# FlinkML/flink-parameter-server

Hardware: NVIDIA H100
Metric: matrix-factorization updates/sec (whole box, max over ranks) (higher is better)
Workload: dtype fp32

## Files before the change

### flink-parameter-server_b200/models/mf/device.py

```python
from __future__ import annotations

import math
import os
from typing import Iterable, Optional, Sequence, Tuple

import torch
import torch.distributed as dist

from ...errors import FactorIsNotANumberException
from ...ops import native
from ...utils.metrics import GLOBAL as METRICS
from ...runtime.device_stream import DevicePrefetcher
from ...store.replica_cache import ReplicaCache
from ...store.sharded_table import ShardedTable

ERR_SIGMOID = 0
ERR_PLAIN = 1

DEFAULT_DEVICE_PULL_LIMIT = 0

L2_TABLE_BYTES = 48 << 20
WINDOW_BUDGET = 256 << 20
WINDOW_BYTES_PER_ROW = 8 + 12
WINDOW_MAX_STRIDE = 128
# ... 89 lines not shown
                 output_ring=None, loss: str = "pointwise", regularization: float = 0.0,
                 step_window: Optional[int] = None, optimizer: str = "sgd",
                 negative_sampling: str = "uniform", margin: Optional[float] = None):
        self._pending = []
        self.step_window = 0
        check_negative_sampling(negative_sampling, negative_sample_rate)
        self.negative_sampling = negative_sampling
        if loss not in ("pointwise", "bpr", "warp"):
            raise ValueError(f"loss must be 'pointwise', 'bpr' or 'warp', got {loss!r}")
        self.loss, self.reg = loss, float(regularization)
        if loss == "pointwise" and self.reg != 0.0:
            raise ValueError("regularization is only supported with loss='bpr' or loss='warp'")
        self.margin = check_warp(loss, margin, optimizer=optimizer, negative_sampling=negative_sampling)
        if loss != "pointwise":
            if output_ring is not None:
                raise ValueError(f"the per-update output ring is not supported with loss={loss!r}")
            if kernel == "tma":
                raise ValueError(f"kernel='tma' is not supported with loss={loss!r}")
            if item_blocking:
                raise ValueError(f"item_blocking is not supported with loss={loss!r}")
            item_blocking = False
        self.device = torch.cuda.current_device() if device is None else int(device)
        self.cuda_device = torch.device("cuda", self.device)
        self.group = group
        ready = dist.is_available() and dist.is_initialized()
        self.world = dist.get_world_size(group) if ready else 1
        self.rank = dist.get_rank(group) if ready else 0
        if item_cache is None:
            item_cache = self.world > 1 and os.environ.get("FPS_ITEM_CACHE", "1") != "0"
        check_optimizer(optimizer, item_cache=bool(item_cache), output_ring=output_ring, kernel=kernel)
        self.optimizer = optimizer
        self.num_users, self.num_items, self.k = int(num_users), int(num_items), int(num_factors)
        self.lr = float(learning_rate)
        self.neg = int(negative_sample_rate)
        self.pull_limit = int(pull_limit)
        self.err_mode = int(err_mode)
        self.seed = int(seed)
        self.step_no = 0
        self.kernel = kernel
        self.credits = (torch.tensor([self.pull_limit, 0], dtype=torch.int32, device=self.cuda_device)
                        if self.pull_limit >= 32 and os.environ.get("FPS_STATIC_LIMITER", "0") != "1"
                        and loss == "pointwise" and optimizer == "sgd" else None)
        self.output_ring = output_ring
        with torch.cuda.device(self.device):
            self._items = ShardedTable(num_items, num_factors, partition="hash", group=group,
                                      device=self.device, init="uniform",
                                      init_range=(range_min, range_max), seed=seed * 2 + 1,
                                      track_touched=track_touched)
            n_local = -(-self.num_users // self.world)
            self._users = torch.empty((n_local, self._items.stride), dtype=torch.float32,
                                     device=self.cuda_device)
            native.init_rows(self._users, self.k, self.rank, self.world, native.PART_HASH, n_local,
                             seed * 2 + 2, range_min, range_max)
            self._stats = torch.zeros(STATS_SIZE[loss], dtype=torch.float32, device=self.cuda_device)
            self._user_acc = self._item_acc = None
            if optimizer == "adagrad":
                self._user_acc = torch.zeros(n_local, dtype=torch.float32, device=self.cuda_device)
                self._item_acc = self._items.row_accumulators()
            self._nan_flag = torch.zeros(1, dtype=torch.int32, device=self.cuda_device)
            self.user_memory = int(user_memory) if self.neg > 0 else 0
            if self.user_memory > 0:
                self.seen = torch.full((n_local, self.user_memory), -1, dtype=torch.int32,
                                       device=self.cuda_device)
                self.seen_pos = torch.zeros(n_local, dtype=torch.int32, device=self.cuda_device)
            self._registry = (native.seen_registry(self.num_items, self.cuda_device)
                              if negative_sampling == "seen" else None)
        self.item_cache = bool(item_cache)
        self.sync_every = max(1, int(sync_every))
        self.sync_interval_ms = sync_interval_ms
        self.flush_count, self.flush_require = flush_count, flush_require
        self._own_inplace = replica_own_inplace
        self.replica = (ReplicaCache(self._items, self.sync_every, sync_interval_ms,
                                     require=flush_require, flush_count=flush_count,
                                     own_inplace=replica_own_inplace)
                        if self.item_cache else None)
        row_bytes = self._items.stride * 4
        if item_blocking is None:
            item_blocking = ((self.world == 1 or self.item_cache) and self.num_items * row_bytes > (48 << 20)
                             and (self.neg == 0 or self.user_memory > 0 or negative_sampling == "seen")
                             and os.environ.get("FPS_ITEM_BLOCKING", "1") != "0")
        self.item_blocking = bool(item_blocking)
        block_bytes = int(os.environ.get("FPS_BLOCK_BYTES", block_bytes))
        self.l2_hints = self.item_blocking and os.environ.get("FPS_L2_HINTS", "0") == "1"
        per_bucket = max(1, int(block_bytes) // row_bytes)
        self.block_shift = max(0, per_bucket.bit_length() - 1)
        table_rows = self._items.rows_per_shard * self.world if self.item_cache else self.num_items
        self._table_rows = table_rows
        while -(-table_rows >> self.block_shift) > native.BUCKET_MAX:
            self.block_shift += 1
        self.block_buckets = max(1, -(-table_rows >> self.block_shift))
        if self.item_blocking:
            with torch.cuda.device(self.device):
                self._bucket_scratch = torch.zeros(2 * native.BUCKET_MAX, dtype=torch.int32,
                                                   device=self.cuda_device)
        self.step_window = step_window_size(step_window, world=self.world, item_cache=self.item_cache,
                                            loss=self.loss, table_rows=self.num_items, stride=self._items.stride,
                                            env=os.environ.get("FPS_STEP_WINDOW"), optimizer=optimizer)
        self._win = None
        self._win_phase_ns = None
        self._graph_capture = False
        self._per_launch = False
        self._items.barrier()

    @property
    def stats(self) -> torch.Tensor:
        self._drain()
        return self._stats

    @property
    def users(self) -> torch.Tensor:
        self._drain()
        return self._users

    @property
    def items(self) -> ShardedTable:
        self._drain()
        return self._items

    @property
    def nan_flag(self) -> torch.Tensor:
        self._drain()
        return self._nan_flag

    @property
    def accumulators(self) -> Optional[Tuple[torch.Tensor, torch.Tensor]]:
        self._drain()
        if self._item_acc is None:
            return None
        return self._user_acc, self._item_acc.local

    def _windowable(self, users, items, ratings) -> bool:
        if self.step_window < 2 or self._graph_capture or self._per_launch:
            return False
        packed = items is None
        return step_windowable(
            neg=self.neg, output_ring=self.output_ring, pull_limit=self.pull_limit, credits=self.credits,
            kernel=self.kernel, kernel_env=os.environ.get("FPS_MF_KERNEL", "reg"),
            reg_variant_env=os.environ.get("FPS_MF_REG_VARIANT"), l2_hints=self.l2_hints, packed=packed,
            dtypes=(users.dtype,) if packed else (users.dtype, items.dtype, ratings.dtype),
            n_records=users.numel(), table_rows=self.num_items, on_gpu=users.is_cuda,
            capturing=torch.cuda.is_current_stream_capturing())

    def _stage(self, users, items, ratings) -> None:
        if self._win is None:
            rows, w = self.num_items, self.step_window
            slot_bytes = -(-rows * 12 // 256) * 256
            with torch.cuda.device(self.device):
                dev = self.cuda_device
                self._win = {
                    "slot_bytes": slot_bytes,
                    "stage": torch.empty(w * slot_bytes, dtype=torch.uint8, device=dev),
                    "slots": torch.full((w, rows), -1, dtype=torch.int64, device=dev),
                    "user_bits": torch.zeros(-(-self._users.shape[0] // 32), dtype=torch.int32, device=dev),
                    "ctl": torch.zeros(2 * native.WINDOW_MAX, dtype=torch.int32, device=dev),
                    "slot_stats": torch.zeros((w, 2), dtype=torch.float32, device=dev),
                }
        j = len(self._pending)
        n = users.numel()
        sb = self._win["slot_bytes"]
        slot = self._win["stage"][j * sb:(j + 1) * sb]
        if items is None:
            slot[:8 * n].view(torch.int64).copy_(users.reshape(-1), non_blocking=True)
        else:
            ids = slot[:12 * n].view(torch.int32)
            ids[:n].copy_(users.reshape(-1), non_blocking=True)
            ids[n:2 * n].copy_(items.reshape(-1), non_blocking=True)
            ids[2 * n:].view(torch.float32).copy_(ratings.reshape(-1), non_blocking=True)
        self._pending.append((n, 1 if items is None else 0))
        self.step_no += 1
        METRICS.inc("mf_ratings", n)

    def _drain(self) -> int:
        n = len(self._pending)
        if n == 0:
            return 0
        counts, fmts = zip(*self._pending)
        self._pending = []
        w = self._win
        native.mf_window_drain(w["stage"], w["slot_bytes"], counts, fmts, self._users, self._items.local, self.lr,
                               self.err_mode, w["slots"], w["user_bits"], w["ctl"], self._stats, w["slot_stats"],
                               self._nan_flag, phase_ns=self._win_phase_ns)
        return n

    def flush(self) -> None:
        self._drain()
        if self.replica is not None:
            self.replica.flush()

    def step(self, users: torch.Tensor, items: Optional[torch.Tensor] = None,
             ratings: Optional[torch.Tensor] = None, negatives: Optional[torch.Tensor] = None) -> None:
        if self.loss == "pointwise" and negatives is None and self._windowable(users, items, ratings):
            self._stage(users, items, ratings)
            if len(self._pending) >= self.step_window:
                self._drain()
            return
        self._drain()
        check_negative_sampling(self.negative_sampling, self.neg, negatives)
        if self.loss != "pointwise":
            self._step_pairwise(users, items, ratings, negatives)
            return
        if negatives is not None:
            raise ValueError("negatives= needs loss='bpr' or loss='warp'")
        neg = self.neg
        if self.user_memory > 0 or self._registry is not None:
            users, items, ratings = self._sample_negatives(users, items, ratings)
            neg = 0
        n_records = users.numel()
        fed = False
        ring = self.output_ring
        out_args = ring.kernel_args() if ring is not None else None
        revisits = self.item_cache or n_records * (1 + neg) > self._table_rows
        if self.item_blocking and self.block_buckets > 1 and revisits:
            hashed = self.item_cache and self._items.mode == native.PART_HASH
            fed = hashed
            users, items, ratings = native.bucket_by_item(
                users, items, ratings, self.block_shift, self.block_buckets, self._bucket_scratch,
                num_shards=self.world if hashed else 1, rows_per_shard=self._items.rows_per_shard,
                pending=self.replica.pending if hashed else None)
        if self.item_cache:
            self.replica.after_step(n_records * (1 + neg), fed=fed)
            native.mf_sgd_fused(users, items, ratings, self._users, self.world, self.replica.table_c,
                                self.lr, err_mode=self.err_mode, neg_rate=neg,
                                num_items=self.num_items, seed=self.seed, step=self.step_no,
                                stats=self._stats, nan_flag=self._nan_flag,
                                max_inflight_rows=self.pull_limit, kernel="reg", l2_hints=self.l2_hints,
                                reserve_total=self.replica.reserve_total(), output=out_args,
                                credits=self.credits)
        else:
            native.mf_sgd_fused(users, items, ratings, self._users, self.world, self._items.table_c,
                                self.lr, err_mode=self.err_mode, neg_rate=neg,
                                num_items=self.num_items, seed=self.seed, step=self.step_no,
                                stats=self._stats, nan_flag=self._nan_flag,
                                max_inflight_rows=self.pull_limit, kernel=self.kernel,
                                l2_hints=self.l2_hints, output=out_args, credits=self.credits,
                                item_acc=self._item_acc.table_c if self._item_acc is not None else None,
                                user_acc=self._user_acc)
        if ring is not None:
            ring.after_kernel(users.numel() * (1 + neg))
        self.step_no += 1
        METRICS.inc("mf_ratings", users.numel())

    def _step_pairwise(self, users, items, ratings, negatives) -> None:
        if negatives is not None:
            if self.item_cache:
                raise ValueError("negatives= is not supported in the replica (item_cache) mode")
            n = int(negatives.shape[1]) if negatives.dim() == 2 else 0
        elif self.neg < 1:
            raise ValueError(f"loss={self.loss!r} needs negative_sample_rate >= 1 or explicit negatives=")
        elif self.user_memory > 0 or self._registry is not None:
            per = 1 + self.neg
            ou, oi, orat = self._sample_negatives(users, items, ratings)
            ou, oi = ou.view(-1, per), oi.view(-1, per)
            negatives = torch.where(ou[:, 1:] >= 0, oi[:, 1:], torch.full_like(oi[:, 1:], -1)).contiguous()
            users, items, ratings = ou[:, 0].contiguous(), oi[:, 0].contiguous(), orat.view(-1, per)[:, 0].contiguous()
            n = self.neg
        else:
            n = self.neg
        if self.output_ring is not None:
            raise ValueError(f"the per-update output ring is not supported with loss={self.loss!r}")
        n_pos = users.numel()
        cand, reserve = self._items.table_c, 0
        if self.item_cache:
            self.replica.after_step(n_pos * (n if self.loss == "bpr" else 1), fed=False)
            cand, reserve = self.replica.table_c, self.replica.reserve_total()
        if self.loss == "warp":
            native.mf_warp_fused(users, items, ratings, self._users, cand, self.lr, self.reg, margin=self.margin,
                                 rank_items=self.num_items, negatives=negatives, n_neg=n, num_items=self.num_items,
                                 seed=self.seed, step=self.step_no, anchor_div=self.world, stats=self._stats,
                                 nan_flag=self._nan_flag, max_inflight_rows=self.pull_limit, reserve_total=reserve)
            self.step_no += 1
            METRICS.inc("mf_ratings", n_pos)
            return
        native.mf_bpr_fused(users, items, ratings, self._users, cand, self.lr, self.reg, negatives=negatives,
                            n_neg=n, num_items=self.num_items, seed=self.seed, step=self.step_no,
                            anchor_div=self.world, stats=self._stats, nan_flag=self._nan_flag,
                            max_inflight_rows=self.pull_limit, reserve_total=reserve,
                            anchor_acc=self._user_acc,
                            cand_acc=self._item_acc.table_c if self._item_acc is not None else None)
        self.step_no += 1
        METRICS.inc("mf_ratings", n_pos)

    def _sample_negatives(self, users, items, ratings):
        memory = self.user_memory > 0
        if self._registry is not None:
            return native.neg_sample_seen(users, items, ratings, self.neg, self._registry,
                                          self.seen if memory else None, self.seen_pos if memory else None,
                                          self.world, seed=self.seed, step=self.step_no)
        return native.neg_sample(users, items, ratings, self.neg, self.num_items, self.seen, self.seen_pos,
                                 self.world, seed=self.seed, step=self.step_no)

    def seen_items(self) -> torch.Tensor:
        if self._registry is None:
            raise ValueError("seen_items() needs negative_sampling='seen'")
        order, count, _ = self._registry
        return order[:int(count.item())].to(torch.int64)

    def make_graph_step(self, batch_size: int, packed: bool = True):
        self._drain()
        dev = self.cuda_device
        if packed:
            static = (torch.zeros(batch_size, dtype=torch.int64, device=dev),)
        else:
            static = (torch.zeros(batch_size, dtype=torch.int32, device=dev),
                      torch.zeros(batch_size, dtype=torch.int32, device=dev),
                      torch.zeros(batch_size, dtype=torch.float32, device=dev))
        s = torch.cuda.Stream(device=dev)
        s.wait_stream(torch.cuda.current_stream(dev))
# ... 127 lines not shown
```

### flink-parameter-server_b200/ops/csrc/fps_mf_window.cu

```cuda
#include <cuda_fp16.h>
#include <cooperative_groups.h>
#include "fps_common.cuh"
#include "fps_mf_args.cuh"

namespace cg = cooperative_groups;

#define WIN_MAX 8
#define WIN_THREADS 256
#define WIN_EMPTY 0xFFFFFFFFFFFFFFFFull

struct WinArgs {
  const unsigned char* stage;
  long long slot_bytes;
  long long n[WIN_MAX];
  int fmt[WIN_MAX];
  int n_slots;
  int err_mode;
  float lr;
  int stride;
  float* user_table;
  float* item_table;
  long long rows;
  unsigned long long* slots;
  unsigned int* user_bits;
  long long bm_words;
  unsigned int* ctl;
  float* stats;
  float* slot_stats;
  int* nan_flag;
  unsigned long long* phase_ns;
};

__device__ __forceinline__ bool win_record(const WinArgs& a, int j, long long i, int& user, int& item,
                                           float& rating) {
  const unsigned char* base = a.stage + (long long)j * a.slot_bytes;
  if (a.fmt[j] == 1) {
    const unsigned long long rec = reinterpret_cast<const unsigned long long*>(base)[i];
    user = (int)(rec >> 38);
    item = (int)((rec >> 16) & 0x3FFFFFull);
    rating = __half2float(__ushort_as_half((unsigned short)(rec & 0xFFFFull)));
    return true;
  }
  const long long n = a.n[j];
  user = reinterpret_cast<const int*>(base)[i];
  item = reinterpret_cast<const int*>(base)[n + i];
  rating = reinterpret_cast<const float*>(base)[2 * n + i];
  return user >= 0;
}

__device__ __forceinline__ float win_add(float x, float y) {
  float z;
  asm("add.rn.ftz.f32 %0, %1, %2;" : "=f"(z) : "f"(x), "f"(y));
  return z;
}
__device__ __forceinline__ float4 win_add4(float4 x, float g, float4 y) {
  return make_float4(win_add(x.x, g * y.x), win_add(x.y, g * y.y), win_add(x.z, g * y.z), win_add(x.w, g * y.w));
}

__device__ __forceinline__ unsigned long long win_clock() {
  unsigned long long t;
  asm volatile("mov.u64 %0, %%globaltimer;" : "=l"(t));
  return t;
}
__device__ __forceinline__ void win_phase(const WinArgs& a, int k) {
  const unsigned long long t = win_clock();
  a.phase_ns[k] += t - a.phase_ns[3];
  a.phase_ns[3] = t;
  if (k == 1) a.phase_ns[2] += 1ull;
}

template <int G, int NS>
__device__ __forceinline__ void win_flush_stats(const WinArgs& a, float (&sq)[NS], float (&cnt)[NS], int nr,
                                                int slot0, float* sh) {
  const int lane = threadIdx.x & (G - 1);
  __syncthreads();
  if (threadIdx.x < 2 * WIN_MAX) sh[threadIdx.x] = 0.f;
  __syncthreads();
#pragma unroll
  for (int r = 0; r < WIN_MAX; ++r) {
    if (r < nr) {
      const bool mine = lane == r % G;
      float s = mine ? sq[r / G] : 0.f, c = mine ? cnt[r / G] : 0.f;
#pragma unroll
      for (int o = 16; o > 0; o >>= 1) {
        s += __shfl_xor_sync(0xffffffffu, s, o);
        c += __shfl_xor_sync(0xffffffffu, c, o);
      }
      if ((threadIdx.x & 31) == 0 && c > 0.f) {
        atomicAdd(sh + 2 * r, s);
        atomicAdd(sh + 2 * r + 1, c);
      }
    }
  }
#pragma unroll
  for (int i = 0; i < NS; ++i) sq[i] = cnt[i] = 0.f;
  __syncthreads();
  if (threadIdx.x < 2 * nr && sh[threadIdx.x] != 0.f)
    atomicAdd(a.slot_stats + 2 * slot0 + threadIdx.x, sh[threadIdx.x]);
}

template <int G, int VPL>
__device__ __forceinline__ void win_load(float4 (&x)[VPL], const float* row, int lane, int nvec, bool on) {
#pragma unroll
  for (int k = 0; k < VPL; ++k) {
    const int c = lane + k * G;
    x[k] = (on && c < nvec) ? *reinterpret_cast<const float4*>(row + 4 * c) : make_float4(0.f, 0.f, 0.f, 0.f);
  }
}
template <int G, int VPL>
__device__ __forceinline__ void win_store(float* row, const float4 (&x)[VPL], int lane, int nvec) {
#pragma unroll
  for (int k = 0; k < VPL; ++k) {
    const int c = lane + k * G;
    if (c < nvec) *reinterpret_cast<float4*>(row + 4 * c) = x[k];
  }
}
template <int G, int VPL>
__device__ __forceinline__ float win_dot(const float4 (&u)[VPL], const float4 (&v)[VPL]) {
  float d[VPL];
#pragma unroll
  for (int k = 0; k < VPL; ++k) {
    d[k] = 0.f;
    d[k] += fps_mf_dot4(u[k], v[k]);
  }
#pragma unroll
  for (int h = VPL / 2; h > 0; h >>= 1)
#pragma unroll
    for (int k = 0; k < h; ++k) d[k] += d[k + h];
  return fps_group_sum<G>(d[0]);
}

template <int LPR, int VPL, int P, int MINB>
__global__ void __launch_bounds__(WIN_THREADS, MINB) fps_mf_window_kernel(const __grid_constant__ WinArgs a) {
  static_assert(VPL >= 1 && VPL <= LPR && LPR % VPL == 0, "VPL must divide LPR");
  constexpr int G = LPR / VPL;
  __shared__ float sh[2 * WIN_MAX];
  cg::grid_group grid = cg::this_grid();
  const int lane = threadIdx.x & (G - 1);
  const int gtid = blockIdx.x * blockDim.x + threadIdx.x;
  const int gthreads = gridDim.x * blockDim.x;
  const int group = gtid / G;
  const int n_groups = gthreads / G;
  const int stride = a.stride;
  const int nvec = stride >> 2;
  constexpr int NS = G < WIN_MAX ? WIN_MAX / G : 1;
  constexpr int NE = NS;
  float sq[NS], cnt[NS];
#pragma unroll
  for (int i = 0; i < NS; ++i) sq[i] = cnt[i] = 0.f;
  bool bad = false;
  const bool timer = a.phase_ns != nullptr && blockIdx.x == 0 && threadIdx.x == 0;

  if (blockIdx.x == 0) {
    if (threadIdx.x < 2 * WIN_MAX) a.ctl[threadIdx.x] = 0u;
    if (threadIdx.x < 2 * a.n_slots) a.slot_stats[threadIdx.x] = 0.f;
  }
  if (timer) a.phase_ns[3] = win_clock();
  int start = 0, attempt = 0;
  while (start < a.n_slots) {
    for (long long w = gtid; w < a.bm_words; w += gthreads) a.user_bits[w] = 0u;
    grid.sync();
    int end = start;
    bool clashed = false;
    while (end < a.n_slots) {
      const int j = end;
      unsigned long long* t = a.slots + (long long)(j - start) * a.rows;
      bool clash = false;
      for (long long i = gtid; i < a.n[j]; i += gthreads) {
        int user, item;
        float rating;
        if (!win_record(a, j, i, user, item, rating)) continue;
        const unsigned long long e = ((unsigned long long)__float_as_uint(rating) << 32) | (unsigned int)user;
        clash |= atomicExch(t + item, e) != WIN_EMPTY;
        const unsigned int bit = 1u << (user & 31);
        clash |= (atomicOr(a.user_bits + (user >> 5), bit) & bit) != 0u;
      }
      if (clash) *reinterpret_cast<volatile unsigned int*>(a.ctl + attempt) = 1u;
      grid.sync();
      clashed = *reinterpret_cast<volatile unsigned int*>(a.ctl + attempt) != 0u;
      ++attempt;
      if (clashed) break;
      ++end;
    }
    if (timer) win_phase(a, 0);
    const int nrow = end - start;
    const int written = nrow + (clashed ? 1 : 0);
    if (nrow > 0) {
      unsigned long long nxt[NE];
#pragma unroll
      for (int m = 0; m < NE; ++m) {
        const int r = lane + m * G;
        nxt[m] = (group < a.rows && r < written) ? a.slots[(long long)r * a.rows + group] : WIN_EMPTY;
      }
      for (long long base = 0; base < a.rows; base += n_groups) {
        const long long item = base + group;
        const bool in = item < a.rows;
        float* vp = a.item_table + (in ? item : 0) * (long long)stride;
        float4 v[VPL];
#pragma unroll
        for (int k = 0; k < VPL; ++k) v[k] = make_float4(0.f, 0.f, 0.f, 0.f);
        bool any = false;
        bool loaded = false;
        unsigned long long mine[NE];
#pragma unroll
        for (int m = 0; m < NE; ++m) {
          const int r = lane + m * G;
          mine[m] = nxt[m];
          const long long it2 = item + n_groups;
          nxt[m] = (it2 < a.rows && r < written) ? a.slots[(long long)r * a.rows + it2] : WIN_EMPTY;
          if (mine[m] != WIN_EMPTY) a.slots[(long long)r * a.rows + item] = WIN_EMPTY;
        }
        const int src0 = (threadIdx.x & 31) & ~(G - 1);
#pragma unroll
        for (int c0 = 0; c0 < WIN_MAX; c0 += P) {
          if (c0 < nrow) {
            unsigned long long ent[P];
#pragma unroll
            for (int q = 0; q < P; ++q) {
              const int r = c0 + q;
              ent[q] = __shfl_sync(0xffffffffu, mine[(r / G) % NE], src0 + r % G);
              if (r >= nrow) ent[q] = WIN_EMPTY;
            }
            {
              bool chunk_any = false;
#pragma unroll
              for (int q = 0; q < P; ++q) chunk_any |= ent[q] != WIN_EMPTY;
              if (chunk_any && !loaded) win_load<G, VPL>(v, vp, lane, nvec, true);
              loaded |= chunk_any;
              any |= chunk_any;
              float4 u[P][VPL];
#pragma unroll
              for (int q = 0; q < P; ++q)
                win_load<G, VPL>(u[q], a.user_table + (long long)(unsigned int)ent[q] * stride, lane, nvec,
                                 ent[q] != WIN_EMPTY);
#pragma unroll
              for (int q = 0; q < P; ++q) {
                const int r = c0 + q;
                if (r < nrow) {
                  const float d = win_dot<G, VPL>(u[q], v);
                  const bool ok = ent[q] != WIN_EMPTY;
                  const float rating = __uint_as_float((unsigned int)(ent[q] >> 32));
                  const float resid = rating - d;
                  const float g = fps_mf_grad(a.err_mode, a.lr, rating, d, resid);
                  if (ok) {
                    if (!(fabsf(g) <= 3.0e38f)) bad = true;
                    if (lane == r % G) {
                      sq[r / G] += resid * resid;
                      cnt[r / G] += 1.f;
                    }
                    float4 nu[VPL];
#pragma unroll
                    for (int k = 0; k < VPL; ++k) {
                      nu[k] = win_add4(u[q][k], g, v[k]);
                      v[k] = win_add4(v[k], g, u[q][k]);
                    }
                    win_store<G, VPL>(a.user_table + (long long)(unsigned int)ent[q] * stride, nu, lane, nvec);
                  }
                }
              }
            }
          }
        }
        if (any) win_store<G, VPL>(vp, v, lane, nvec);
      }
      win_flush_stats<G, NS>(a, sq, cnt, nrow, start, sh);
    } else {
      const int j = start;
      unsigned long long* t = a.slots;
      for (long long base = 0; base < a.n[j]; base += n_groups) {
        const long long i = base + group;
        int user = 0, item = 0;
        float rating = 0.f;
        const bool ok = i < a.n[j] && win_record(a, j, i, user, item, rating);
        float* up = a.user_table + (long long)user * stride;
        float* vp = a.item_table + (long long)item * stride;
        float4 u[VPL], v[VPL];
#pragma unroll
        for (int k = 0; k < VPL; ++k) {
          const int c = lane + k * G;
          u[k] = v[k] = make_float4(0.f, 0.f, 0.f, 0.f);
          if (ok && c < nvec) {
            v[k] = fps_ld_row4(vp + 4 * c);
            u[k] = *reinterpret_cast<const float4*>(up + 4 * c);
          }
        }
        const float d = win_dot<G, VPL>(u, v);
        const float resid = rating - d;
        const float g = fps_mf_grad(a.err_mode, a.lr, rating, d, resid);
        if (ok) {
          if (!(fabsf(g) <= 3.0e38f)) bad = true;
          if (lane == 0) {
            sq[0] += resid * resid;
            cnt[0] += 1.f;
            t[item] = WIN_EMPTY;
          }
#pragma unroll
          for (int k = 0; k < VPL; ++k) {
            const int c = lane + k * G;
            if (c < nvec) {
              fps_red_add4(up + 4 * c, make_float4(g * v[k].x, g * v[k].y, g * v[k].z, g * v[k].w));
              fps_red_add4(vp + 4 * c, make_float4(g * u[k].x, g * u[k].y, g * u[k].z, g * u[k].w));
            }
          }
        }
      }
      win_flush_stats<G, NS>(a, sq, cnt, 1, start, sh);
      end = start + 1;
    }
    grid.sync();
    if (timer) win_phase(a, 1);
    start = end;
  }
  if (bad && a.nan_flag != nullptr) *a.nan_flag = 1;
  if (blockIdx.x == 0 && threadIdx.x == 0 && a.stats != nullptr) {
    float s = 0.f, c = 0.f;
    for (int j = 0; j < a.n_slots; ++j) {
      s += a.slot_stats[2 * j];
      c += a.slot_stats[2 * j + 1];
    }
    a.stats[0] += s;
    a.stats[1] += c;
  }
}

template <int LPR, int VPL, int P, int MINB>
static int launch_window(const WinArgs& a, int num_sms, cudaStream_t stream) {
  constexpr int V = VPL < LPR ? VPL : LPR;
  int occ = 0;
  cudaError_t e =
      cudaOccupancyMaxActiveBlocksPerMultiprocessor(&occ, fps_mf_window_kernel<LPR, V, P, MINB>, WIN_THREADS, 0);
  if (e != cudaSuccess) return (int)e;
  if (occ < 1) return -1402;
  const long long grid = (long long)num_sms * occ;
  WinArgs args = a;
  void* params[] = {&args};
  e = cudaLaunchCooperativeKernel((const void*)fps_mf_window_kernel<LPR, V, P, MINB>, dim3((unsigned)grid),
                                  dim3(WIN_THREADS), params, 0, stream);
  if (e != cudaSuccess) return (int)e;
  return (int)cudaGetLastError();
}

static int g_win_variant = 0;
extern "C" void fps_set_mf_window_variant(int v) { g_win_variant = v; }

template <int LPR>
static int dispatch_window(const WinArgs& a, int num_sms, cudaStream_t s) {
  constexpr int MINB_V1 = LPR <= 2 ? 2 : 3;
  switch (g_win_variant) {
    case 1: return launch_window<LPR, 1, 8, 1>(a, num_sms, s);
    case 2: return launch_window<LPR, 1, 4, MINB_V1>(a, num_sms, s);
    default:
      if constexpr (LPR == 16) return launch_window<16, 4, 2, 2>(a, num_sms, s);
      else return launch_window<LPR, 1, 4, MINB_V1>(a, num_sms, s);
  }
}

extern "C" int fps_mf_window_drain(const WinArgs* a, int num_sms, cudaStream_t stream) {
  if (a->n_slots <= 0) return 0;
  if (a->n_slots > WIN_MAX) return -1401;
  const int nvec = a->stride >> 2;
  if (nvec <= 1) return dispatch_window<1>(*a, num_sms, stream);
  if (nvec <= 2) return dispatch_window<2>(*a, num_sms, stream);
  if (nvec <= 4) return dispatch_window<4>(*a, num_sms, stream);
  if (nvec <= 8) return dispatch_window<8>(*a, num_sms, stream);
  if (nvec <= 16) return dispatch_window<16>(*a, num_sms, stream);
  if (nvec <= 32) return dispatch_window<32>(*a, num_sms, stream);
  return -1400;
}
```

### flink-parameter-server_b200/ops/native.py

```python
from __future__ import annotations

import ctypes as C
import math
import os
import threading
from typing import Optional

import torch

from . import build as _build

FPS_MAX_SHARDS = 16
PART_HASH = 0
PART_RANGE = 1
PART_LUT = 2
LUT_OWNER_SHIFT = 40

_lib = None
_lib_lock = threading.Lock()
_launch_count = 0


class ShardTableC(C.Structure):

# ... 138 lines not shown
    _check(lib().fps_heap_free(C.c_void_p(ptr)), "heap_free")


def ipc_get_handle(ptr: int) -> bytes:
    buf = (C.c_ubyte * 64)()
    _check(lib().fps_ipc_get_handle(C.c_void_p(ptr), buf), "ipc_get_handle")
    return bytes(buf)


def ipc_open_handle(handle: bytes) -> int:
    buf = (C.c_ubyte * 64).from_buffer_copy(handle)
    out = C.c_void_p()
    _check(lib().fps_ipc_open_handle(buf, C.byref(out)), "ipc_open_handle")
    return int(out.value)


def ipc_close(ptr: int) -> None:
    _check(lib().fps_ipc_close(C.c_void_p(ptr)), "ipc_close")


def enable_peer(dev: int, peer: int) -> None:
    _check(lib().fps_enable_peer(int(dev), int(peer)), f"enable_peer({dev},{peer})")


class _RawCudaBuffer:

    def __init__(self, ptr: int, shape, typestr: str):
        self.__cuda_array_interface__ = {
            "shape": tuple(shape),
            "typestr": typestr,
            "data": (int(ptr), False),
            "version": 3,
            "strides": None,
        }


_TYPESTR = {torch.float32: "<f4", torch.int32: "<i4", torch.int64: "<i8", torch.uint8: "|u1",
            torch.float16: "<f2", torch.int16: "<i2"}


def tensor_from_ptr(ptr: int, shape, dtype: torch.dtype, device: int) -> torch.Tensor:
    if dtype == torch.bfloat16:
        t = torch.as_tensor(_RawCudaBuffer(ptr, shape, "<i2"), device=torch.device("cuda", device))
        return t.view(torch.bfloat16)
    return torch.as_tensor(_RawCudaBuffer(ptr, shape, _TYPESTR[dtype]),
                           device=torch.device("cuda", device))


def init_rows(rows: torch.Tensor, dim: int, shard: int, num_shards: int, mode: int, div: int,
              seed: int, lo: float, hi: float) -> None:
    _req(rows, "rows", torch.float32)
    n_rows, stride = rows.shape
    assert stride % 4 == 0
    _check(lib().fps_init_rows(C.c_void_p(rows.data_ptr()), C.c_longlong(n_rows), int(dim),
                               int(stride), int(shard), int(num_shards), int(mode),
                               C.c_longlong(div), C.c_ulonglong(seed & (2**64 - 1)),
                               C.c_float(lo), C.c_float(hi), _stream()), "init_rows")
    _bump()


def mf_sgd_fused(users: torch.Tensor, items: torch.Tensor, ratings: torch.Tensor,
                 user_table, user_div: int, item_tab: ShardTableC, lr: float,
                 err_mode: int = 0, neg_rate: int = 0, num_items: int = 0, seed: int = 0,
                 step: int = 0, stats: Optional[torch.Tensor] = None,
                 nan_flag: Optional[torch.Tensor] = None, max_inflight_rows: int = 0,
                 kernel: Optional[str] = None, push_tab: Optional[ShardTableC] = None,
                 l2_hints: bool = False, reserve_ctas: int = 0, reserve_total: int = 0,
                 progress: Optional[torch.Tensor] = None, output=None,
                 credits: Optional[torch.Tensor] = None, item_acc: Optional[ShardTableC] = None,
                 user_acc=None) -> None:
    _req(users, "users")
    user_sharded = isinstance(user_table, ShardTableC)
    if not user_sharded:
        _req(user_table, "user_table", torch.float32)
    packed = items is None
    if packed:
        if users.dtype != torch.int64:
            raise TypeError("packed rating records must be an int64 tensor (see pack_ratings)")
    else:
        _req(items, "items"); _req(ratings, "ratings", torch.float32)
        if users.dtype != items.dtype:
            raise TypeError("users and items must share an integer dtype")
    if (user_table.stride if user_sharded else user_table.shape[1]) != item_tab.stride:
        raise ValueError("user table stride must equal item table stride")
    a = MfArgsC()
    a.users = users.data_ptr()
    a.items = None if packed else items.data_ptr()
    a.ratings = None if packed else ratings.data_ptr()
    a.format = 1 if packed else 0
    a.n_pos = users.numel(); a.neg_rate = int(neg_rate); a.num_items = int(max(num_items, 1))
    a.seed = seed & (2**64 - 1); a.step = int(step)
    if user_sharded:
        a.user_table = None; a.user_tab = user_table; a.user_sharded = 1
    else:
        a.user_table = user_table.data_ptr(); a.user_sharded = 0
    a.user_div = int(user_div)
    a.user_shift = log2_or_neg(int(user_div))
    a.lr = float(lr); a.err_mode = int(err_mode)
    a.stats = stats.data_ptr() if stats is not None else None
    a.nan_flag = nan_flag.data_ptr() if nan_flag is not None else None
    a.item_tab = item_tab
    if push_tab is not None:
        a.push_tab = push_tab; a.use_push_tab = 1
    a.l2_hints = 1 if l2_hints else 0
    variant = kernel or os.environ.get("FPS_MF_KERNEL", "reg")
    if packed or push_tab is not None or l2_hints or output is not None or credits is not None:
        variant = "reg"
    a.progress = progress.data_ptr() if progress is not None else None
    if credits is not None:
        _req(credits, "credits", torch.int32)
        a.credits = credits.data_ptr()
    if output is not None:
        o_ids, o_vecs, o_staged, o_cap, o_every = output
        a.out_ids = o_ids.data_ptr(); a.out_vecs = o_vecs.data_ptr(); a.out_staged = o_staged.data_ptr()
        a.out_cap = int(o_cap); a.out_every = int(o_every)
    if item_acc is not None:
        if push_tab is not None or output is not None or credits is not None:
            raise ValueError("row-wise AdaGrad does not support push_tab, output or credits")
        if int(item_acc.stride) != 1:
            raise ValueError("item_acc must be a stride-1 accumulator table")
        a.item_acc = item_acc
        if user_sharded:
            if not isinstance(user_acc, ShardTableC) or int(user_acc.stride) != 1:
                raise ValueError("a sharded user table needs a stride-1 ShardTableC user_acc")
            a.user_acc_tab = user_acc
        else:
            if not torch.is_tensor(user_acc):
                raise ValueError("a worker-local user table needs a float32 user_acc tensor")
            _req(user_acc, "user_acc", torch.float32)
            if user_acc.numel() < user_table.shape[0]:
                raise ValueError("user_acc must hold one accumulator per user row")
            a.user_acc = user_acc.data_ptr()
        variant = "reg"
    elif user_acc is not None:
        raise ValueError("user_acc needs item_acc")
    lib().fps_set_mf_reserve(int(reserve_ctas))
    lib().fps_set_mf_reserve_total(int(reserve_total))
    rv = os.environ.get("FPS_MF_REG_VARIANT")
    if rv is not None:
        lib().fps_set_mf_reg_variant(int(rv))
    if variant == "tma":
        code = lib().fps_mf_sgd_tma(C.byref(a), _id_bytes(users), int(max_inflight_rows),
                                    sm_count(users.device.index), _stream())
        if code != -1002:
            _check(code, "mf_sgd_tma")
            _bump()
            return
    _check(lib().fps_mf_sgd_fused(C.byref(a), 4 if packed else _id_bytes(users), int(max_inflight_rows),
                                  sm_count(users.device.index), _stream()), "mf_sgd_fused")
    _bump()


WINDOW_MAX = 8


class WinArgsC(C.Structure):

    _fields_ = [
        ("stage", C.c_void_p), ("slot_bytes", C.c_longlong),
        ("n", C.c_longlong * WINDOW_MAX), ("fmt", C.c_int * WINDOW_MAX),
        ("n_slots", C.c_int), ("err_mode", C.c_int), ("lr", C.c_float), ("stride", C.c_int),
        ("user_table", C.c_void_p), ("item_table", C.c_void_p), ("rows", C.c_longlong),
        ("slots", C.c_void_p), ("user_bits", C.c_void_p), ("bm_words", C.c_longlong),
        ("ctl", C.c_void_p), ("stats", C.c_void_p), ("slot_stats", C.c_void_p), ("nan_flag", C.c_void_p),
        ("phase_ns", C.c_void_p),
    ]


def mf_window_drain(stage: torch.Tensor, slot_bytes: int, counts, formats, user_table: torch.Tensor,
                    item_table: torch.Tensor, lr: float, err_mode: int, slots: torch.Tensor,
                    user_bits: torch.Tensor, ctl: torch.Tensor, stats: torch.Tensor, slot_stats: torch.Tensor,
                    nan_flag: torch.Tensor, phase_ns: Optional[torch.Tensor] = None) -> None:
    n = len(counts)
    if not 0 < n <= WINDOW_MAX or len(formats) != n:
        raise ValueError(f"1..{WINDOW_MAX} staged micro-batches expected, got {n}")
    for t, name in ((stage, "stage"), (user_table, "user_table"), (item_table, "item_table"), (slots, "slots"),
                    (user_bits, "user_bits"), (ctl, "ctl"), (stats, "stats"), (slot_stats, "slot_stats"),
                    (nan_flag, "nan_flag")):
        _req(t, name)
    if user_table.shape[1] != item_table.shape[1]:
        raise ValueError("user table stride must equal item table stride")
    if user_bits.numel() * 32 < user_table.shape[0] or slots.numel() < n * item_table.shape[0]:
        raise ValueError("user bitmap or slot table too small")
    if slot_stats.numel() < 2 * n or ctl.numel() < 2 * WINDOW_MAX:
        raise ValueError("slot_stats / ctl too small")
    a = WinArgsC()
    a.stage = stage.data_ptr(); a.slot_bytes = int(slot_bytes)
    for j in range(n):
        a.n[j] = int(counts[j]); a.fmt[j] = int(formats[j])
    a.n_slots = n; a.err_mode = int(err_mode); a.lr = float(lr); a.stride = int(item_table.shape[1])
    a.user_table = user_table.data_ptr(); a.item_table = item_table.data_ptr(); a.rows = int(item_table.shape[0])
    a.slots = slots.data_ptr(); a.user_bits = user_bits.data_ptr(); a.bm_words = user_bits.numel()
    a.ctl = ctl.data_ptr(); a.stats = stats.data_ptr(); a.slot_stats = slot_stats.data_ptr()
    a.nan_flag = nan_flag.data_ptr()
    if phase_ns is not None:
        _req(phase_ns, "phase_ns", torch.int64)
        if phase_ns.numel() < 4:
            raise ValueError("phase_ns too small")
        a.phase_ns = phase_ns.data_ptr()
    rv = os.environ.get("FPS_MF_WINDOW_VARIANT")
    if rv is not None:
        lib().fps_set_mf_window_variant(int(rv))
    _check(lib().fps_mf_window_drain(C.byref(a), sm_count(stage.device.index), _stream()), "mf_window_drain")
    _bump()


class BprArgsC(C.Structure):

    _fields_ = [
        ("users", C.c_void_p), ("items", C.c_void_p), ("ratings", C.c_void_p), ("negatives", C.c_void_p),
        ("n_pos", C.c_longlong), ("n_neg", C.c_int), ("format", C.c_int),
        ("num_items", C.c_longlong), ("seed", C.c_ulonglong), ("step", C.c_ulonglong),
        ("lr", C.c_float), ("reg", C.c_float),
        ("anchor_table", C.c_void_p), ("anchor_div", C.c_int), ("anchor_shift", C.c_int),
        ("anchor_sharded", C.c_int), ("cand_sharded", C.c_int), ("anchor_tab", ShardTableC),
        ("cand_table", C.c_void_p), ("cand_div", C.c_int), ("cand_shift", C.c_int), ("cand_tab", ShardTableC),
        ("use_push_tab", C.c_int), ("stride", C.c_int), ("push_tab", ShardTableC),
        ("stats", C.c_void_p), ("nan_flag", C.c_void_p), ("reserve_total", C.c_int), ("pad_", C.c_int),
        ("anchor_acc_tab", ShardTableC), ("cand_acc", ShardTableC), ("anchor_acc", C.c_void_p),
        ("rank_items", C.c_longlong), ("margin", C.c_float), ("pad2_", C.c_int),
    ]


def _pairwise_args(users, items, ratings, anchor_table, cand_table, lr, reg, negatives, n_neg, num_items, seed,
                   step, anchor_div, cand_div, stats, n_stats, nan_flag, push_tab, reserve_total):
    _req(users, "users")
    packed = items is None
    if packed:
        if users.dtype != torch.int64:
            raise TypeError("packed rating records must be an int64 tensor (see pack_ratings)")
        id_dtype = torch.int32
    else:
        _req(items, "items"); _req(ratings, "ratings", torch.float32)
        if users.dtype != items.dtype:
            raise TypeError("users and items must share an integer dtype")
        if items.numel() != users.numel() or ratings.numel() != users.numel():
            raise ValueError("users, items and ratings must have the same length")
        id_dtype = users.dtype
    n_pos = users.numel()
    a = BprArgsC()
    strides = []
    for name, tab, div in (("anchor", anchor_table, anchor_div), ("cand", cand_table, cand_div)):
        if isinstance(tab, ShardTableC):
            setattr(a, f"{name}_tab", tab); setattr(a, f"{name}_sharded", 1)
            strides.append(int(tab.stride))
        else:
            _req(tab, f"{name}_table", torch.float32)
            setattr(a, f"{name}_table", tab.data_ptr())
            setattr(a, f"{name}_div", int(div)); setattr(a, f"{name}_shift", log2_or_neg(int(div)))
            strides.append(int(tab.shape[1]))
    if strides[0] != strides[1]:
        raise ValueError("anchor table stride must equal candidate table stride")
    a.stride = strides[0]
    if push_tab is not None:
        if not a.cand_sharded:
            raise ValueError("push_tab needs a ShardTable cand_table")
        if int(push_tab.stride) != a.stride:
            raise ValueError("push table stride must equal candidate table stride")
        a.push_tab = push_tab; a.use_push_tab = 1
    if negatives is not None:
        _req(negatives, "negatives", id_dtype)
        if negatives.dim() != 2 or negatives.shape[0] != n_pos:
            raise ValueError(f"negatives must be [{n_pos}, n]")
        a.negatives = negatives.data_ptr(); a.n_neg = int(negatives.shape[1])
    else:
        if int(n_neg) < 1:
            raise ValueError("n_neg must be >= 1 when negatives are sampled")
        a.n_neg = int(n_neg)
    if stats is not None:
        _req(stats, "stats", torch.float32)
        if stats.numel() < n_stats:
            raise ValueError(f"stats must hold {n_stats} floats")
        a.stats = stats.data_ptr()
    if nan_flag is not None:
        _req(nan_flag, "nan_flag", torch.int32)
        a.nan_flag = nan_flag.data_ptr()
    a.users = users.data_ptr()
    a.items = None if packed else items.data_ptr()
    a.ratings = None if packed else ratings.data_ptr()
    a.format = 1 if packed else 0
    a.n_pos = n_pos; a.num_items = int(max(num_items, 1))
    a.seed = seed & (2**64 - 1); a.step = int(step)
    a.lr = float(lr); a.reg = float(reg); a.reserve_total = int(reserve_total)
    return a, packed


def mf_bpr_fused(users: torch.Tensor, items: Optional[torch.Tensor], ratings: Optional[torch.Tensor],
                 anchor_table, cand_table, lr: float, reg: float = 0.0, *,
                 negatives: Optional[torch.Tensor] = None, n_neg: int = 1, num_items: int = 0,
                 seed: int = 0, step: int = 0, anchor_div: int = 1, cand_div: int = 1,
                 stats: Optional[torch.Tensor] = None, nan_flag: Optional[torch.Tensor] = None,
                 max_inflight_rows: int = 0, push_tab: Optional[ShardTableC] = None,
                 reserve_total: int = 0, anchor_acc=None, cand_acc: Optional[ShardTableC] = None) -> None:
    a, packed = _pairwise_args(users, items, ratings, anchor_table, cand_table, lr, reg, negatives, n_neg, num_items,
                               seed, step, anchor_div, cand_div, stats, 3, nan_flag, push_tab, reserve_total)
    if cand_acc is not None:
        if not a.cand_sharded or push_tab is not None:
            raise ValueError("row-wise AdaGrad needs a ShardTableC cand_table and no push_tab")
        if int(cand_acc.stride) != 1:
            raise ValueError("cand_acc must be a stride-1 accumulator table")
        a.cand_acc = cand_acc
        if a.anchor_sharded:
            if not isinstance(anchor_acc, ShardTableC) or int(anchor_acc.stride) != 1:
                raise ValueError("a sharded anchor table needs a stride-1 ShardTableC anchor_acc")
            a.anchor_acc_tab = anchor_acc
        else:
            if not torch.is_tensor(anchor_acc):
                raise ValueError("a worker-local anchor table needs a float32 anchor_acc tensor")
            _req(anchor_acc, "anchor_acc", torch.float32)
            if anchor_acc.numel() < anchor_table.shape[0]:
                raise ValueError("anchor_acc must hold one accumulator per anchor row")
            a.anchor_acc = anchor_acc.data_ptr()
    elif anchor_acc is not None:
        raise ValueError("anchor_acc needs cand_acc")
    _check(lib().fps_mf_bpr_fused(C.byref(a), 4 if packed else _id_bytes(users), int(max_inflight_rows),
                                  sm_count(users.device.index), _stream()), "mf_bpr_fused")
    _bump()


WARP_TRIAL_BLOCKS = (1, 2, 4, 8)


def mf_warp_fused(users: torch.Tensor, items: Optional[torch.Tensor], ratings: Optional[torch.Tensor],
                  anchor_table, cand_table, lr: float, reg: float = 0.0, *, margin: float = 1.0,
                  rank_items: int = 0, negatives: Optional[torch.Tensor] = None, n_neg: int = 1,
                  num_items: int = 0, seed: int = 0, step: int = 0, anchor_div: int = 1, cand_div: int = 1,
                  stats: Optional[torch.Tensor] = None, nan_flag: Optional[torch.Tensor] = None,
                  max_inflight_rows: int = 0, push_tab: Optional[ShardTableC] = None, reserve_total: int = 0,
                  trial_block: int = 0) -> None:
    if not math.isfinite(float(margin)):
        raise ValueError(f"margin must be finite, got {margin!r}")
    if int(trial_block) not in (0,) + WARP_TRIAL_BLOCKS:
        raise ValueError(f"trial_block must be 0 or one of {WARP_TRIAL_BLOCKS}, got {trial_block!r}")
    a, packed = _pairwise_args(users, items, ratings, anchor_table, cand_table, lr, reg, negatives, n_neg, num_items,
                               seed, step, anchor_div, cand_div, stats, 4, nan_flag, push_tab, reserve_total)
    a.margin = float(margin)
    a.rank_items = int(rank_items) if int(rank_items) > 0 else int(a.num_items)
# ... 770 lines not shown
```

Baseline: 3.360 billion.

## Scatter all window slots optimistically before one grid sync, fall back on clash

The window drain kernel now scatters every staged micro-batch into the slot tables in a single pass and uses one grid-wide sync to check for item or user clashes. Previously each slot was scattered with its own grid sync. When nothing clashes, the whole window is applied as one batch. On a clash, a slow-path flag clears the slots and reruns the old slot-by-slot scan. The user bitmap is now cleared at kernel exit instead of at the start of each pass. This cuts grid.sync calls in the common no-clash case, at the cost of wasted scatter work and an extra clear whenever clashes happen.

Result: faster. 3.399 billion, median of 6 (+1.2%).

```diff
diff --git a/flink-parameter-server_b200/models/mf/device.py b/flink-parameter-server_b200/models/mf/device.py
--- a/flink-parameter-server_b200/models/mf/device.py
+++ b/flink-parameter-server_b200/models/mf/device.py
@@ -265,7 +265,7 @@
                     "stage": torch.empty(w * slot_bytes, dtype=torch.uint8, device=dev),
                     "slots": torch.full((w, rows), -1, dtype=torch.int64, device=dev),
                     "user_bits": torch.zeros(-(-self._users.shape[0] // 32), dtype=torch.int32, device=dev),
-                    "ctl": torch.zeros(2 * native.WINDOW_MAX, dtype=torch.int32, device=dev),
+                    "ctl": torch.zeros(native.WINDOW_CTL, dtype=torch.int32, device=dev),
                     "slot_stats": torch.zeros((w, 2), dtype=torch.float32, device=dev),
                 }
         j = len(self._pending)
diff --git a/flink-parameter-server_b200/ops/csrc/fps_mf_window.cu b/flink-parameter-server_b200/ops/csrc/fps_mf_window.cu
--- a/flink-parameter-server_b200/ops/csrc/fps_mf_window.cu
+++ b/flink-parameter-server_b200/ops/csrc/fps_mf_window.cu
@@ -8,6 +8,7 @@
 #define WIN_MAX 8
 #define WIN_THREADS 256
 #define WIN_EMPTY 0xFFFFFFFFFFFFFFFFull
+#define WIN_CTL (2 * WIN_MAX + 1)
 
 struct WinArgs {
   const unsigned char* stage;
@@ -48,6 +49,20 @@
   return user >= 0;
 }
 
+__device__ __forceinline__ bool win_scatter(const WinArgs& a, int j, unsigned long long* t, int gtid, int gthreads) {
+  bool clash = false;
+  for (long long i = gtid; i < a.n[j]; i += gthreads) {
+    int user, item;
+    float rating;
+    if (!win_record(a, j, i, user, item, rating)) continue;
+    const unsigned long long e = ((unsigned long long)__float_as_uint(rating) << 32) | (unsigned int)user;
+    clash |= atomicExch(t + item, e) != WIN_EMPTY;
+    const unsigned int bit = 1u << (user & 31);
+    clash |= (atomicOr(a.user_bits + (user >> 5), bit) & bit) != 0u;
+  }
+  return clash;
+}
+
 __device__ __forceinline__ float win_add(float x, float y) {
   float z;
   asm("add.rn.ftz.f32 %0, %1, %2;" : "=f"(z) : "f"(x), "f"(y));
@@ -156,31 +171,37 @@
     if (threadIdx.x < 2 * a.n_slots) a.slot_stats[threadIdx.x] = 0.f;
   }
   if (timer) a.phase_ns[3] = win_clock();
+  volatile unsigned int* slow = a.ctl + WIN_CTL - 1;
+  {
+    bool clash = false;
+    for (int j = 0; j < a.n_slots; ++j) clash |= win_scatter(a, j, a.slots + (long long)j * a.rows, gtid, gthreads);
+    if (clash) *slow = 1u;
+  }
+  grid.sync();
+  if (*slow != 0u) {
+#pragma unroll 1
+    for (long long w = gtid; w < (long long)a.n_slots * a.rows; w += gthreads) a.slots[w] = WIN_EMPTY;
+  }
   int start = 0, attempt = 0;
   while (start < a.n_slots) {
-    for (long long w = gtid; w < a.bm_words; w += gthreads) a.user_bits[w] = 0u;
-    grid.sync();
     int end = start;
     bool clashed = false;
-    while (end < a.n_slots) {
-      const int j = end;
-      unsigned long long* t = a.slots + (long long)(j - start) * a.rows;
-      bool clash = false;
-      for (long long i = gtid; i < a.n[j]; i += gthreads) {
-        int user, item;
-        float rating;
-        if (!win_record(a, j, i, user, item, rating)) continue;
-        const unsigned long long e = ((unsigned long long)__float_as_uint(rating) << 32) | (unsigned int)user;
-        clash |= atomicExch(t + item, e) != WIN_EMPTY;
-        const unsigned int bit = 1u << (user & 31);
-        clash |= (atomicOr(a.user_bits + (user >> 5), bit) & bit) != 0u;
-      }
-      if (clash) *reinterpret_cast<volatile unsigned int*>(a.ctl + attempt) = 1u;
+    if (*slow == 0u) {
+      end = a.n_slots;
+    } else {
+#pragma unroll 1
+      for (long long w = gtid; w < a.bm_words; w += gthreads) a.user_bits[w] = 0u;
       grid.sync();
-      clashed = *reinterpret_cast<volatile unsigned int*>(a.ctl + attempt) != 0u;
-      ++attempt;
-      if (clashed) break;
-      ++end;
+      while (end < a.n_slots) {
+        const int j = end;
+        const bool clash = win_scatter(a, j, a.slots + (long long)(j - start) * a.rows, gtid, gthreads);
+        if (clash) *reinterpret_cast<volatile unsigned int*>(a.ctl + attempt) = 1u;
+        grid.sync();
+        clashed = *reinterpret_cast<volatile unsigned int*>(a.ctl + attempt) != 0u;
+        ++attempt;
+        if (clashed) break;
+        ++end;
+      }
     }
     if (timer) win_phase(a, 0);
     const int nrow = end - start;
@@ -311,6 +332,9 @@
     if (timer) win_phase(a, 1);
     start = end;
   }
+#pragma unroll 1
+  for (long long w = gtid; w < a.bm_words; w += gthreads) a.user_bits[w] = 0u;
+  if (blockIdx.x == 0 && threadIdx.x == 0) *slow = 0u;
   if (bad && a.nan_flag != nullptr) *a.nan_flag = 1;
   if (blockIdx.x == 0 && threadIdx.x == 0 && a.stats != nullptr) {
     float s = 0.f, c = 0.f;
diff --git a/flink-parameter-server_b200/ops/native.py b/flink-parameter-server_b200/ops/native.py
--- a/flink-parameter-server_b200/ops/native.py
+++ b/flink-parameter-server_b200/ops/native.py
@@ -314,6 +314,7 @@
 
 
 WINDOW_MAX = 8
+WINDOW_CTL = 2 * WINDOW_MAX + 1
 
 
 class WinArgsC(C.Structure):
@@ -344,7 +345,7 @@
         raise ValueError("user table stride must equal item table stride")
     if user_bits.numel() * 32 < user_table.shape[0] or slots.numel() < n * item_table.shape[0]:
         raise ValueError("user bitmap or slot table too small")
-    if slot_stats.numel() < 2 * n or ctl.numel() < 2 * WINDOW_MAX:
+    if slot_stats.numel() < 2 * n or ctl.numel() < WINDOW_CTL:
         raise ValueError("slot_stats / ctl too small")
     a = WinArgsC()
     a.stage = stage.data_ptr(); a.slot_bytes = int(slot_bytes)
```
